# mitschabaude/msm-zprize

Measured on AMD Instinct MI355X. Metric: Mpoint-adds/s (ms per MSM in ms_per_step), higher is better.
Workload: dtype u32 limbs (28-bit lazy Montgomery, i64 accumulate)

## Files before the change

msm_zprize_amd/csrc/batch_kernels.h:

```cpp
#pragma once

namespace msmz {

#ifndef MSMZ_BATCH_BMAX
#define MSMZ_BATCH_BMAX 16
#endif
#ifdef MSMZ_EXP_NOMUL
#define BM_MUL(r, a, b) fe_add(r, a, b)
#define BM_SQR(r, a) fe_add(r, a, a)
#else
#define BM_MUL(r, a, b) fe_mul(r, a, b)
#define BM_SQR(r, a) fe_sqr(r, a)
#endif
enum { PK_NONE = 0, PK_ADD = 1, PK_DBL = 2, PK_TAKE_A = 3, PK_TAKE_B = 4, PK_INF = 5 };

template <class F, int T, bool SAFE, int OCC, int BMAX>
__global__ void __launch_bounds__(T, OCC) k_batch_add(uint32_t* slots, const uint32_t* points, const uint2* dsc,
                                                      uint32_t out_base, uint32_t total, int B, MsmMeta* meta) {
  __shared__ int32_t tree[F::N * T];
  __shared__ int32_t s_prev[F::N * T];
  __shared__ uint8_t s_kind[SAFE ? BMAX * T : 1];
  constexpr int N = F::N;
  const uint32_t block_base = blockIdx.x * (uint32_t)(T * B);
#ifdef MSMZ_TRACE
  uint64_t* trace = reinterpret_cast<uint64_t*>(meta + 1);
#endif
  MSMZ_STAMP(trace, 0);
  MSMZ_STAMP_HW(trace);

  Fe<F> prefix;
  fe_set_const<F>(prefix, F::ONE);
  int ilast = -1;
  if (block_base + threadIdx.x < total) {
    const uint32_t room = (total - 1u - block_base - threadIdx.x) / (uint32_t)T;
    ilast = room < (uint32_t)(B - 1) ? (int)room : B - 1;
  }
  uint2 dnext = make_uint2(0, 0);
  if (block_base + threadIdx.x < total) dnext = dsc[block_base + threadIdx.x];
#pragma unroll 1
  for (int i = 0; i < B; i++) {
    const uint32_t t = block_base + (uint32_t)i * T + threadIdx.x;
    uint32_t kind = PK_NONE;
    uint2 dd = dnext;
    if (i + 1 < B && t + (uint32_t)T < total) dnext = dsc[t + (uint32_t)T];
    if (t < total) {
#if defined(MSMZ_EXP_LOCALMEM) || defined(MSMZ_EXP_LOCAL_FWD)
      dd.x = LOC_ORIG | (t & 4095u);
      dd.y = LOC_ORIG | ((t + 1u) & 4095u);
#endif
      Fe<F> d;
      kind = PK_ADD;
      if constexpr (SAFE && SlotFmt<F>::PACKED) {
        Fe<F> x1, x2;
        const uint32_t oa = load_operand_x_or<F>(x1, dd.x, slots, points);
        const uint32_t ob = load_operand_x_or<F>(x2, dd.y, slots, points);
        fe_sub(d, x2, x1);
        if (oa == 0 || ob == 0 || fe_is_zero(d)) {
          Affine<F> p1, p2;
          const bool infA = load_operand<F, true>(p1, dd.x, slots, points);
          const bool infB = load_operand<F, true>(p2, dd.y, slots, points);
          if (infA) {
            kind = infB ? PK_INF : PK_TAKE_B;
          } else if (infB) {
            kind = PK_TAKE_A;
          } else if (fe_is_zero(d)) {
            Fe<F> num;
            fe_sub(num, p2.y, p1.y);
            if (fe_is_zero(num) && !fe_is_zero(p1.y)) {
              kind = PK_DBL;
              fe_add(d, p2.y, p2.y);
            } else {
// ... 208 lines not shown
```

msm_zprize_amd/csrc/engine.h:

```cpp
#pragma once
#include <hip/hip_runtime.h>

#include <chrono>
#include <cstdio>
#include <cstdlib>
#include <cstring>
#include <map>
#include <type_traits>
#include <vector>

#include "../../include/msmz.h"
#include "kernels.h"
#include "gen_kernels.h"
#include "import_kernels.h"
#include "check_kernels.h"
#include "mul_kernels.h"
#include "host64.h"
#include "multi.h"
#include "plan.h"

namespace msmz {

#define MSMZ_HIP(x)                                                                        \
  do {                                                                                     \
// ... 6 lines not shown

struct DevBuf {
  void* p = nullptr;
  size_t bytes = 0;
  DevBuf() = default;
  DevBuf(DevBuf&& o) noexcept : p(o.p), bytes(o.bytes) { o.p = nullptr, o.bytes = 0; }
  DevBuf& operator=(DevBuf&& o) noexcept {
    if (this != &o) {
      release();
      p = o.p, bytes = o.bytes;
      o.p = nullptr, o.bytes = 0;
    }
    return *this;
  }
  DevBuf(const DevBuf&) = delete;
  DevBuf& operator=(const DevBuf&) = delete;
  ~DevBuf() { release(); }
  int ensure(size_t need) {
    if (need <= bytes) return MSMZ_OK;
    release();
    size_t sz = need + need / 8;
    if (hipMalloc(&p, sz) != hipSuccess) {
      if (hipMalloc(&p, need) != hipSuccess) return MSMZ_ERR_HIP;
      sz = need;
    }
    bytes = sz;
    return MSMZ_OK;
  }
  void release() {
    if (p) (void)hipFree(p);
    p = nullptr;
    bytes = 0;
  }
  template <class T>
  T* as() const {
    return reinterpret_cast<T*>(p);
  }
};

struct Handle {
  int kind;
  uint64_t n;
  bool has_endo;
  DevBuf mem;
  uint32_t factor = 0;
  int c = 0, glv = 0;
  uint64_t copy_stride = 0;
  int sbits = 0;
};

struct StageEvents {
  hipEvent_t sort0, hist_end, scan_end, coarse_end, sort_end;
  hipEvent_t plan0, plan_end;
  hipEvent_t round_end[32];
  hipEvent_t acc_end, red_end;
  std::vector<hipEvent_t*> all() {
    std::vector<hipEvent_t*> v{&sort0, &hist_end, &scan_end, &coarse_end, &sort_end, &plan0, &plan_end, &acc_end, &red_end};
    for (hipEvent_t& e : round_end) v.push_back(&e);
    return v;
  }
};

struct Run {
  bool timing = false;
  StageEvents ev{};
  uint32_t max_bucket = 0, n_entries = 0, rounds = 0;
  uint32_t round_pairs[32] = {}, round_base[32] = {};
  uint64_t n_pairs = 0;
};

enum class Redo { NONE, PROVEN_BITS, PER_PROBLEM };

template <class F, bool TE>
static int host_point_add(const uint8_t* a, int ai, const uint8_t* b, int bi, uint8_t* out, int* oi) {
  constexpr int NW = F::NW;
  if constexpr (TE) {
    auto load = [](TeExt<F>& p, const uint8_t* xy) {
      uint32_t w[2 * NW];
      memcpy(w, xy, sizeof(w));
      Fe<F> x, y;
      fe_unpack<F>(x, w);
      fe_unpack<F>(y, w + NW);
      fe_to_mont(p.X, x);
      fe_to_mont(p.Y, y);
      fe_set_const<F>(p.Z, F::ONE);
      fe_mul(p.T, p.X, p.Y);
    };
    if (!a || !b) return MSMZ_ERR_ARG;
    TeExt<F> p, q, r;
    load(p, a);
    load(q, b);
    te_add(r, p, q);
    uint32_t w[2 * NW];
    te_to_affine_canon<F>(w, r);
    memcpy(out, w, sizeof(w));
    *oi = 0;
  } else {
    auto load = [](Xyzz<F>& p, const uint8_t* xy, int inf) {
      if (inf) {
        xyzz_set_inf(p);
        return;
      }
      uint32_t w[2 * NW];
      memcpy(w, xy, sizeof(w));
      Affine<F> t, m;
      fe_unpack<F>(t.x, w);
      fe_unpack<F>(t.y, w + NW);
      fe_to_mont(m.x, t.x);
      fe_to_mont(m.y, t.y);
      xyzz_from_affine(p, m);
    };
    Xyzz<F> p, q, r;
    load(p, a, ai);
    load(q, b, bi);
    xyzz_add(r, p, q);
    uint32_t w[2 * NW];
    bool inf = xyzz_to_affine_canon<F>(w, r);
    memcpy(out, w, sizeof(w));
    *oi = inf ? 1 : 0;
  }
  return MSMZ_OK;
}

struct ReduceKnobs {
  uint32_t tail_n;
  uint32_t quad16_max;
  uint32_t pairsum_x4_max;
};

template <class Cfg>
class TestHooks;

template <class Cfg>
class Engine : public IEngine {
  friend class TestHooks<Cfg>;
  using F = typename Cfg::F;
  using Fr = typename Cfg::Fr;
  static constexpr int NW = F::NW;
  static constexpr int RW = 2 * NW;
  static constexpr int XW = 4 * NW;
  static constexpr int FE_BYTES = NW * 4;
  static constexpr bool TE = Cfg::TE;
  static constexpr int PW_WORDS = TE ? 4 * NW : PointFmt<F>::STRIDE;

 public:
  Engine(int curve_id, int device) : curve_id_(curve_id), device_(device) {}

  int init() {
    MSMZ_HIP(hipSetDevice(device_));
    MSMZ_HIP(hipStreamCreateWithFlags(&stream_, hipStreamNonBlocking));
    for (hipEvent_t* e : ev_.all()) MSMZ_HIP(hipEventCreate(e));
    MSMZ_HIP(hipEventCreateWithFlags(&import_ev_, hipEventDisableTiming));
    MSMZ_HIP(hipHostMalloc(&h_meta_, sizeof(MsmMeta)));
    int st;
    if ((st = ensure_host_results((size_t)2 * kMaxWindows * XW))) return st;
    if ((st = raise_lds_limit((const void*)k_fine, "k_fine", kFineLds))) return st;
    if ((st = raise_sort_limits<false, 0>()) || (st = raise_sort_limits<false, 16>()) || (st = raise_sort_limits<false, 17>())) return st;
    if constexpr (Fr::HAS_GLV) {
      if ((st = raise_sort_limits<true, 0>()) || (st = raise_sort_limits<true, 16>())) return st;
    }
    return meta_.ensure(sizeof(MsmMeta) + kTraceBytes * 65536);
  }
 private:
  template <bool GLV, int C>
  int raise_sort_limits() {
    int st;
    if ((st = raise_lds_limit((const void*)k_coarse<Fr, GLV, C>, GLV ? "k_coarse<glv>" : "k_coarse", kCoarseLdsMax))) return st;
    return raise_lds_limit((const void*)k_hist<Fr, GLV, C>, GLV ? "k_hist<glv>" : "k_hist", kHistLdsMax);
  }
  static constexpr size_t kFineLds = ((size_t)(1 << FINE_MAX_BITS) + FINE_STAGE) * 4;
  static constexpr size_t kCoarseLdsMax = (size_t)2 * SORT_MAX_BINS * 4;
  static constexpr size_t kHistLdsMax = (size_t)SORT_MAX_BINS * 4;
#ifdef MSMZ_TRACE
  static constexpr size_t kTraceBytes = 128;
#else
  static constexpr size_t kTraceBytes = 0;
#endif

#ifdef MSMZ_TRACE
  int trace_dump(const char* name, const void* d_stamps, uint32_t n_wgs, bool first) {
    const char* path = getenv("MSMZ_TRACE_OUT");
    if (!path) return MSMZ_OK;
    MSMZ_HIP(hipStreamSynchronize(stream_));
    std::vector<uint64_t> t((size_t)n_wgs * 16);
    MSMZ_HIP(hipMemcpy(t.data(), d_stamps, t.size() * 8, hipMemcpyDeviceToHost));
    if (FILE* f = fopen(path, first ? "wb" : "ab")) {
      char nm[32] = {};
      strncpy(nm, name, 31);
      const uint64_t n = n_wgs;
      fwrite(nm, 1, 32, f);
      fwrite(&n, 8, 1, f);
      fwrite(t.data(), 8, t.size(), f);
      fclose(f);
    }
    return MSMZ_OK;
  }
#endif

  int raise_lds_limit(const void* fn, const char* name, size_t dyn_max) {
    hipFuncAttributes fa;
    memset(&fa, 0, sizeof(fa));
    MSMZ_HIP(hipFuncGetAttributes(&fa, fn));
    hipDeviceProp_t prop;
    MSMZ_HIP(hipGetDeviceProperties(&prop, device_));
    size_t dev_max = prop.sharedMemPerBlock;
    if (prop.sharedMemPerBlockOptin > dev_max) dev_max = prop.sharedMemPerBlockOptin;
    if (prop.maxSharedMemoryPerMultiProcessor > dev_max) dev_max = prop.maxSharedMemoryPerMultiProcessor;
    if (fa.sharedSizeBytes + dyn_max > dev_max) {
      fprintf(stderr, "msmz: %s needs %zu B static + %zu B dynamic LDS, the device offers %zu B per workgroup\n", name,
              (size_t)fa.sharedSizeBytes, dyn_max, dev_max);
      return MSMZ_ERR_HIP;
    }
    MSMZ_HIP(hipFuncSetAttribute(fn, hipFuncAttributeMaxDynamicSharedMemorySize, (int)dyn_max));
    return MSMZ_OK;
  }

 public:
  ~Engine() override {
    (void)hipSetDevice(device_);
    if (h_meta_) (void)hipHostFree(h_meta_);
    if (h_res_) (void)hipHostFree(h_res_);
    if (h_check_) (void)hipHostFree(h_check_);
    for (hipEvent_t* e : ev_.all())
      if (*e) (void)hipEventDestroy(*e);
    if (import_ev_) (void)hipEventDestroy(import_ev_);
    if (stream_) (void)hipStreamDestroy(stream_);
  }

  int upload_points(const uint8_t* xy, const uint8_t* inf, uint64_t n, uint64_t* h, const GenMap* split = nullptr) override {
    if (!xy || !h || n == 0 || n >= (1ull << (Cfg::HAS_ENDO ? 29 : 30))) return MSMZ_ERR_ARG;
    MSMZ_HIP(hipSetDevice(device_));
    int st = stage_.ensure(n * RW * 4 + n);
    if (st) return st;
    if ((st = copy_h2d(stage_.p, xy, (size_t)RW * 4, n, split))) return st;
    uint8_t* d_inf = nullptr;
    if (inf) {
      d_inf = stage_.as<uint8_t>() + n * RW * 4;
      if ((st = copy_h2d(d_inf, inf, 1, n, split))) return st;
    }
    const bool endo = Cfg::HAS_ENDO;
    Handle hd{0, n, endo};
    if ((st = alloc_handle(hd, (size_t)n * PW_WORDS * 4 * (endo ? 2 : 1)))) return st;
    MsmMeta* d_meta = meta_.as<MsmMeta>();
    MSMZ_HIP(hipMemsetAsync(&d_meta->error, 0, 4, stream_));
    if constexpr (TE) {
      hipLaunchKernelGGL((k_te_points_to_niels<F>), dim3((n + 255) / 256), dim3(256), 0, stream_, hd.mem.as<uint32_t>(),
                         stage_.as<uint32_t>(), (uint32_t)n, &d_meta->error);
    } else {
      hipLaunchKernelGGL((k_points_to_mont<F>), dim3((n + 255) / 256), dim3(256), 0, stream_, hd.mem.as<uint32_t>(),
                         stage_.as<uint32_t>(), d_inf, (uint32_t)n, endo ? 1 : 0, &d_meta->error);
    }
    uint32_t err = 0;
    if ((st = fetch_error(&err))) return st;
    if (err) return MSMZ_ERR_RANGE;
    return add_handle(std::move(hd), h);
  }

  int upload_scalars(const uint8_t* s, uint64_t n, uint64_t* h, const GenMap* split = nullptr) override {
    if (!s || !h || n == 0) return MSMZ_ERR_ARG;
    MSMZ_HIP(hipSetDevice(device_));
    Handle hd{1, n, false};
    int st;
    if ((st = alloc_handle(hd, n * 32)) || (st = copy_h2d(hd.mem.p, s, 32, n, split))) return st;
    MsmMeta* d_meta = meta_.as<MsmMeta>();
    MSMZ_HIP(hipMemsetAsync(&d_meta->error, 0, 4, stream_));
    hipLaunchKernelGGL((k_check_scalars<Fr>), dim3((n + 255) / 256), dim3(256), 0, stream_, &d_meta->error,
                       hd.mem.as<const uint32_t>(), (uint32_t)n);
    uint32_t err = 0;
    if ((st = fetch_error(&err))) return st;
    if (err) return MSMZ_ERR_RANGE;
    return add_handle(std::move(hd), h);
  }

  int import_scalars(const msmz_src& s, uint64_t n, uint64_t* h, const GenMap* split = nullptr) override {
    if (!h || n == 0 || n >> 32) return MSMZ_ERR_ARG;
    MSMZ_HIP(hipSetDevice(device_));
    Handle hd{1, n, false};
    ImportView v;
// ... 667 lines not shown
        hipLaunchKernelGGL(k_fine, dim3(fbins, P), dim3(FINE_T), lds, stream_, refs_.as<uint32_t>(), off_.as<uint32_t>(),
                           &d_meta->max_bucket, packed_.as<uint32_t>(), bins_.as<uint32_t>(), g.fb, g.fbt, sl.fine_top,
                           fbins, g.idx_bits, n_half, pl.endo_delta, g.F, g.mbits, copy_stride);
      }
#ifdef MSMZ_TRACE
      if ((st = trace_dump("k_coarse", tileoff_.as<uint32_t>() + (size_t)P * tiles * nbins, tiles, true))) return st;
      if ((st = trace_dump("k_fine", bins_.as<uint32_t>() + ((P * g.sbins + 2) & ~1u), fbins, false))) return st;
#endif
    } else {
      if (pl.fold_shift != 0) return MSMZ_ERR_ARG;
      if ((st = digits_.ensure((size_t)K * M * 4))) return st;
      if ((st = counts_.ensure(((size_t)nb + 1) * 4))) return st;
      if ((st = cursor_.ensure((size_t)nb * 4))) return st;
      if ((st = partials_.ensure((size_t)32 * nblocks * 4))) return st;
      MSMZ_HIP(hipMemsetAsync(counts_.p, 0, ((size_t)nb + 1) * 4, stream_));
      MSMZ_HIP(hipMemsetAsync(cursor_.p, 0, (size_t)nb * 4, stream_));
      const uint32_t dgrid = (n + 256 * DIGITS_ITEMS - 1) / (256 * DIGITS_ITEMS);
      mark(run, run.ev.sort0);
      if (pl.glv) {
        if constexpr (Fr::HAS_GLV)
          hipLaunchKernelGGL((k_digits<Fr, true>), dim3(dgrid), dim3(256), 0, stream_, digits_.as<uint32_t>(),
                             counts_.as<uint32_t>(), d_meta, d_scalars, n, c, K, pl.spread, pl.sbits ? pl.sbits : 256);
      } else {
        hipLaunchKernelGGL((k_digits<Fr, false>), dim3(dgrid), dim3(256), 0, stream_, digits_.as<uint32_t>(),
                           counts_.as<uint32_t>(), d_meta, d_scalars, n, c, K, pl.spread, pl.sbits ? pl.sbits : 256);
      }
      mark(run, run.ev.hist_end);
      MSMZ_HIP(hipGetLastError());
      hipLaunchKernelGGL(k_scan_partials, dim3(nblocks, 1), dim3(SCAN_T), 0, stream_, partials_.as<uint32_t>(),
                         counts_.as<uint32_t>(), nb, 0, nblocks);
      hipLaunchKernelGGL(k_scan_top, dim3(1), dim3(SCAN_T), 0, stream_, partials_.as<uint32_t>(), nblocks,
                         &d_meta->n_entries);
      hipLaunchKernelGGL(k_scan_apply, dim3(nblocks, 1), dim3(SCAN_T), 0, stream_, off_.as<uint32_t>(),
                         partials_.as<uint32_t>(), counts_.as<uint32_t>(), nb, 0, nblocks, (size_t)0,
                         &d_meta->max_bucket);
      mark(run, run.ev.scan_end);
      MSMZ_HIP(hipGetLastError());
      {
        dim3 grid((M + 256 * 4 - 1) / (256 * 4), K);
        hipLaunchKernelGGL(k_scatter, grid, dim3(256), 0, stream_, refs_.as<uint32_t>(), cursor_.as<uint32_t>(),
                           off_.as<uint32_t>(), digits_.as<uint32_t>(), M, c, pl.spread, n_half, pl.endo_delta);
      }
      mark(run, run.ev.coarse_end);
      MSMZ_HIP(hipGetLastError());
    }
    mark(run, run.ev.sort_end);
    MSMZ_HIP(hipGetLastError());
    return MSMZ_OK;
  }

  int fetch_meta(Run& run) {
    MSMZ_HIP(hipMemcpyAsync(h_meta_, meta_.p, sizeof(MsmMeta), hipMemcpyDeviceToHost, stream_));
    MSMZ_HIP(hipStreamSynchronize(stream_));
    run.max_bucket = h_meta_->max_bucket;
    run.n_entries = h_meta_->n_entries;
    run.rounds = h_meta_->rounds;
    memcpy(run.round_pairs, h_meta_->round_pairs, sizeof(run.round_pairs));
    memcpy(run.round_base, h_meta_->round_base, sizeof(run.round_base));
    return MSMZ_OK;
  }

  template <class P>
  int reduce_levels(const ReduceKnobs& rk, int& cur, uint32_t n_in, uint32_t nprob) {
    constexpr int AW = P::ACC_WORDS;
    int st;
    while (n_in > rk.tail_n) {
      const uint32_t S = 4;
      uint32_t g2 = (n_in + S - 1) / S;
      int nxt = cur ^ 1;
      if ((st = red_[nxt * 2].ensure((size_t)nprob * g2 * AW * 4))) return st;
      if ((st = red_[nxt * 2 + 1].ensure((size_t)nprob * g2 * AW * 4))) return st;
      uint32_t total = nprob * g2;
      if (total <= rk.quad16_max) {
        hipLaunchKernelGGL((k_reduce_quad16<P>), dim3((total * 16 + 63) / 64), dim3(64), 0, stream_,
                           red_[nxt * 2].as<uint32_t>(), red_[nxt * 2 + 1].as<uint32_t>(),
                           red_[cur * 2].as<uint32_t>(), red_[cur * 2 + 1].as<uint32_t>(), n_in, g2, total);
      } else {
        hipLaunchKernelGGL((k_reduce_quad<P>), dim3((total * 4 + 63) / 64), dim3(64), 0, stream_,
                           red_[nxt * 2].as<uint32_t>(), red_[nxt * 2 + 1].as<uint32_t>(),
                           red_[cur * 2].as<uint32_t>(), red_[cur * 2 + 1].as<uint32_t>(), n_in, g2, total);
      }
      n_in = g2;
      cur = nxt;
    }
    {
      const int nxt = cur ^ 1;
      if ((st = red_[nxt * 2].ensure((size_t)nprob * n_in * AW * 4))) return st;
      if ((st = red_[nxt * 2 + 1].ensure((size_t)nprob * n_in * AW * 4))) return st;
      if ((st = final_.ensure((size_t)nprob * AW * 4))) return st;
      hipLaunchKernelGGL((k_reduce_tail<P>), dim3(nprob), dim3(REDUCE_TAIL_T), 0, stream_, red_[cur * 2].as<uint32_t>(),
                         red_[cur * 2 + 1].as<uint32_t>(), red_[nxt * 2].as<uint32_t>(), red_[nxt * 2 + 1].as<uint32_t>(),
                         final_.as<uint32_t>(), n_in, n_in);
    }
    return MSMZ_OK;
  }

  int fetch_window_sums(const Plan& pl, size_t per_problem) {
    const size_t words = pl.nprob * per_problem * XW;
    if (int st = ensure_host_results(words)) return st;
    MSMZ_HIP(hipGetLastError());
    MSMZ_HIP(hipMemcpyAsync(h_res_, final_.p, words * 4, hipMemcpyDeviceToHost, stream_));
    MSMZ_HIP(hipMemcpyAsync(h_meta_, meta_.p, sizeof(MsmMeta), hipMemcpyDeviceToHost, stream_));
    MSMZ_HIP(hipStreamSynchronize(stream_));
    return MSMZ_OK;
  }

  struct HostTe {
    using Pt = TeExt<F>;
    void set_inf(Pt& p) const { te_set_zero(p); }
    void dbl(Pt& r, const Pt& p) const { te_add(r, p, p); }
    void add_pt(Pt& r, const Pt& a, const Pt& b) const { te_add(r, a, b); }
// ... 64 lines not shown
    } else if (basic) {
      hipLaunchKernelGGL((k_reduce2d_partial_acc<P>), dim3((total + 127) / 128), dim3(128), 0, stream_,
                         red_[0].as<uint32_t>(), slots_.as<uint32_t>(), rscan_.as<uint32_t>(), g, total);
    } else {
      if constexpr (!TE)
        hipLaunchKernelGGL((k_reduce2d_partial<F>), dim3((total + 127) / 128), dim3(128), 0, stream_,
                           red_[0].as<uint32_t>(), slots_.as<uint32_t>(), d_points, bfin_.as<uint4>(), g, total);
    }
    int src = 0;
    for (uint32_t n = total / 2; n >= lines && g.NC > 1; n /= 2) {
      const int dst = src ^ 2;
      if (n <= rk.pairsum_x4_max) {
        hipLaunchKernelGGL((k_pairsum_x4<P>), dim3((n * 4 + 63) / 64), dim3(64), 0, stream_, red_[dst].as<uint32_t>(),
                           red_[src].as<uint32_t>(), n);
      } else {
        hipLaunchKernelGGL((k_pairsum<P>), dim3((n + 127) / 128), dim3(128), 0, stream_, red_[dst].as<uint32_t>(),
                           red_[src].as<uint32_t>(), n);
      }
      src = dst;
      if (n == lines) break;
    }
    *rows = src;
    return MSMZ_OK;
  }
  template <class P>
  int weighted_sums_2d(const R2Geom& g, const ReduceKnobs& rk, int crow) {
    const uint32_t lines = g.nprob * g.H;
    const int ccol = crow + 1;
    int st;
    if ((st = red_[ccol].ensure((size_t)lines * XW * 4))) return st;
    hipLaunchKernelGGL((k_fill_neutral<P>), dim3((lines + 255) / 256), dim3(256), 0, stream_, red_[ccol].as<uint32_t>(), lines);
    int cur = crow >> 1;
    if ((st = reduce_levels<P>(rk, cur, g.H, g.nprob))) return st;
    MSMZ_HIP(hipGetLastError());
    return MSMZ_OK;
  }
  static void fill_log(msmz_log* log, const Plan& pl, const Run& run, float host_ms) {
    if (!log) return;
    log->c = pl.c;
    log->K = pl.K;
    log->rounds = (int)run.rounds;
    log->glv = pl.glv ? 1 : 0;
    log->n_entries = run.n_entries;
    log->n_pairs = run.n_pairs;
    log->max_bucket = run.max_bucket;
    log->stage_ms[MSMZ_ST_FINAL] = host_ms;
    if (!run.timing) return;
    const StageEvents& ev = run.ev;
    log->stage_ms[MSMZ_ST_DIGITS] = elapsed(ev.sort0, ev.hist_end);
    log->stage_ms[MSMZ_ST_SCAN] = elapsed(ev.hist_end, ev.scan_end);
    log->stage_ms[MSMZ_ST_SCATTER] = elapsed(ev.scan_end, ev.sort_end);
    log->scatter_kernel_ms = elapsed(ev.scan_end, ev.coarse_end);
    log->scatter_launches = 1;
    log->stage_ms[MSMZ_ST_PLAN] = elapsed(ev.plan0, ev.plan_end);
    log->stage_ms[MSMZ_ST_ACCUMULATE] = elapsed(ev.plan_end, ev.acc_end);
    log->stage_ms[MSMZ_ST_REDUCE] = elapsed(ev.acc_end, ev.red_end);
    hipEvent_t prev = ev.plan_end;
    for (uint32_t r = 0; r < run.rounds && r < 32; r++) {
      if (run.round_pairs[r] == 0) continue;
      log->batch_add_ms[r] = elapsed(prev, ev.round_end[r]);
      prev = ev.round_end[r];
    }
  }

  int plan_phase(const PlanChunks& pc, uint32_t nb, int tail_skip, size_t desc_records, Run& run) {
    int st;
    MsmMeta* d_meta = meta_.as<MsmMeta>();
    mark(run, run.ev.plan0);
    const uint32_t n_chunks = pc.n_main + (nb - pc.nb_main + pc.chunk_top - 1) / pc.chunk_top;
    const size_t pair_words = (size_t)n_chunks * (PLAN_RMAX - PLAN_RL) * PLAN_T;
    if ((st = rscan_.ensure(((size_t)PLAN_RMAX * n_chunks + pair_words) * 4 + kTraceBytes * n_chunks))) return st;
    if ((st = desc_.ensure(desc_records * 8))) return st;
    if ((st = bfin_.ensure((size_t)nb * 16))) return st;
    hipLaunchKernelGGL(k_plan_count, dim3(n_chunks), dim3(PLAN_T), 0, stream_, rscan_.as<uint32_t>(), off_.as<uint32_t>(),
                       nb, n_chunks, d_meta, tail_skip, pc);
    hipLaunchKernelGGL(k_plan_emit, dim3(n_chunks), dim3(PLAN_T), 0, stream_, desc_.as<uint2>(), bfin_.as<uint4>(),
                       d_meta, rscan_.as<uint32_t>(), off_.as<uint32_t>(), refs_.as<uint32_t>(), nb, n_chunks,
                       tail_skip, rscan_.as<uint32_t>() + (size_t)PLAN_RMAX * n_chunks, pc);
    MSMZ_HIP(hipGetLastError());
#ifdef MSMZ_TRACE
    if ((st = trace_dump("k_plan_emit", rscan_.as<uint32_t>() + (size_t)PLAN_RMAX * n_chunks + pair_words, n_chunks, false))) return st;
#endif
    return MSMZ_OK;
  }

  int msm_weierstrass_affine(const Handle& pts, const uint32_t* d_points, const uint32_t* d_scalars, uint64_t n64,
                             const msmz_opts& opt, uint8_t* out, int* out_inf, msmz_log* log, int extra_bits,
                             uint32_t nprob, Redo* redo) {
    const bool glv = opt.glv != 0;
    if (glv && (!Fr::HAS_GLV || !pts.has_endo)) return MSMZ_ERR_UNSUPPORTED;
    Plan pl;
    const bool want_2d = opt.reserved[0] != 1;
    const uint32_t fac = pts.factor > 1 ? pts.factor : 1;
    if (fac > 1 && (!want_2d || glv != (pts.glv != 0))) return MSMZ_ERR_UNSUPPORTED;
    int st = planner_.make_plan(pl, n64, glv, opt, (uint32_t)pts.n, true, extra_bits, want_2d, nprob, fac);
    if (st) return st;
    const SortLayout sl = planner_.sort_layout(pl);
    if (fac > 1 && !sl.two_level) return MSMZ_ERR_ARG;
    if (nprob > 1 && (!want_2d || !sl.two_level)) {
      *redo = Redo::PER_PROBLEM;
      return MSMZ_OK;
    }
    if ((uint64_t)nprob * pl.K * pl.M >= (1ull << 30)) return MSMZ_ERR_ARG;
    const size_t f2_records = opt.reserved[0] == 1 ? (size_t)13 * pl.Keff * ((pl.L + 1) / 2) + 256 : 0;
    if ((st = slots_.ensure(((size_t)nprob * pl.K * pl.M + 64 + f2_records) * SlotFmt<F>::WORDS * 4))) return st;
    Run run = new_run(opt);
    if ((st = sort_phase(pl, sl, d_scalars, run, (uint32_t)pts.copy_stride))) return st;
    const uint32_t nb = pl.nb * nprob;
    MsmMeta* d_meta = meta_.as<MsmMeta>();

    const int tail_skip = want_2d ? tail_skip_2d_ : 0;
    if ((st = plan_phase(planner_.plan_chunks(pl), nb, tail_skip, (size_t)nprob * pl.K * pl.M, run))) return st;
    if ((st = fetch_meta(run))) return st;
    if (h_meta_->error & 4u) return MSMZ_ERR_RANGE;
    if (h_meta_->error & 2u) {
      *redo = Redo::PROVEN_BITS;
      return MSMZ_OK;
    }
    if (run.max_bucket > (pl.F > 1 ? (1u << PLAN_RMAX) - 1u : (1u << 24))) return MSMZ_ERR_ARG;
    mark(run, run.ev.plan_end);
    const uint32_t R = run.rounds;
    for (uint32_t r = 0; r < R; r++) run.n_pairs += run.round_pairs[r];
    for (uint32_t r = 0; r < R; r++) {
      const uint32_t pairs = run.round_pairs[r];
      if (pairs == 0) continue;
      launch_batch_add(pairs, opt.safe != 0, d_points, desc_.as<uint2>() + run.round_base[r], run.round_base[r], d_meta);
#ifdef MSMZ_TRACE
      {
        char nm[32];
        snprintf(nm, sizeof nm, "k_batch_add round %d", r);
        const int B = batch_b(pairs);
        const uint32_t wgs = (pairs + MSMZ_BATCH_T * B - 1) / (MSMZ_BATCH_T * B);
        if ((st = trace_dump(nm, d_meta + 1, wgs < 65536 ? wgs : 65536, false))) return st;
      }
#endif
      mark(run, run.ev.round_end[r]);
    }
    mark(run, run.ev.acc_end);

    if (want_2d) {
      if ((st = reduce_2d<WeierPolicy<F>>(pl, planner_.split_2d(pl), reduce_knobs_, d_points))) return st;
    } else {
      uint32_t S1 = planner_.first_group_size(pl);
      if (S1 > 8) S1 = 8;
      while (S1 > 1 && S1 * 2 > pl.L) S1 >>= 1;
      const uint32_t groups = (pl.L + S1 - 1) / S1;
      if ((st = red_[0].ensure((size_t)pl.Keff * groups * XW * 4))) return st;
      if ((st = red_[1].ensure((size_t)pl.Keff * groups * XW * 4))) return st;
      if ((st = reduce_first_affine(pl, d_points, S1, groups, run.n_pairs, d_meta))) return st;
      int cur = 0;
      if ((st = reduce_levels<WeierPolicy<F>>(reduce_knobs_, cur, groups, (uint32_t)pl.Keff))) return st;
    }
    return finish_msm(pl, run, want_2d, out, out_inf, log);
  }

  int msm_basic(const Handle& pts, const uint32_t* d_points, const uint32_t* d_scalars, uint64_t n64, const msmz_opts& opt,
                uint8_t* out, int* out_inf, msmz_log* log) {
    using P = typename std::conditional<TE, TePolicy<F>, WeierPolicy<F>>::type;
    if (opt.glv) return MSMZ_ERR_UNSUPPORTED;
    Plan pl;
    int st = planner_.make_plan(pl, n64, false, opt, (uint32_t)pts.n, false);
    if (st) return st;
    Run run = new_run(opt);
    if ((st = sort_phase(pl, planner_.sort_layout(pl), d_scalars, run, 0)) || (st = fetch_meta(run))) return st;
    if (h_meta_->error & 4u) return MSMZ_ERR_RANGE;
    run.n_pairs = run.n_entries;
    if ((st = partials_.ensure((size_t)32 * pl.nblocks * 4))) return st;
    constexpr int AW = P::ACC_WORDS;
    const uint32_t nb = pl.nb, nblocks = pl.nblocks;
    MsmMeta* d_meta = meta_.as<MsmMeta>();
    mark(run, run.ev.plan0);
    int chunk_shift = chunk_shift_override_ > 0 ? chunk_shift_override_ : ACC_CHUNK_SHIFT;
    while ((1ull << (2 * chunk_shift)) < run.max_bucket) chunk_shift++;
    const int scan_mode = 2 | (chunk_shift << 4);
    if ((st = rscan_.ensure(((size_t)nb + 1) * 4))) return st;
    hipLaunchKernelGGL(k_scan_partials, dim3(nblocks, 1), dim3(SCAN_T), 0, stream_, partials_.as<uint32_t>(),
                       off_.as<uint32_t>(), nb, scan_mode, nblocks);
    hipLaunchKernelGGL(k_scan_top, dim3(1), dim3(SCAN_T), 0, stream_, partials_.as<uint32_t>(), nblocks,
                       d_meta->round_pairs);
    hipLaunchKernelGGL(k_scan_apply, dim3(nblocks, 1), dim3(SCAN_T), 0, stream_, rscan_.as<uint32_t>(),
                       partials_.as<uint32_t>(), off_.as<uint32_t>(), nb, scan_mode, nblocks, (size_t)0, (uint32_t*)nullptr);
    MSMZ_HIP(hipMemcpyAsync(h_meta_, d_meta, sizeof(MsmMeta), hipMemcpyDeviceToHost, stream_));
    MSMZ_HIP(hipStreamSynchronize(stream_));
    const uint32_t n_chunks = h_meta_->round_pairs[0];
    mark(run, run.ev.plan_end);
    if ((st = slots_.ensure((size_t)(n_chunks + 1) * AW * 4))) return st;
    if (n_chunks > 0) {
      hipLaunchKernelGGL((k_bucket_accumulate<P>), dim3((n_chunks + 127) / 128), dim3(128), 0, stream_,
                         slots_.as<uint32_t>(), d_points, refs_.as<uint32_t>(), off_.as<uint32_t>(),
// ... 25 lines not shown
    g.out0 = g.inf_slot + 64;
    uint32_t n_launch = 0, dsum = 0, osum = 0;
    for (uint32_t step = 1; step < S; step++) {
      g.ppg[n_launch] = 1;
      g.desc_off[n_launch] = dsum;
      g.out_off[n_launch] = osum;
      dsum += g.NG;
      osum += g.NG;
      n_launch++;
    }
    for (uint32_t n = S - 1; n > 1; n = n / 2 + (n & 1)) {
      g.ppg[n_launch] = n / 2;
      g.desc_off[n_launch] = dsum;
      g.out_off[n_launch] = osum;
      dsum += g.NG * (n / 2);
      osum += g.NG * (n / 2);
      n_launch++;
    }
    g.n_launches = n_launch;
    g.desc_off[n_launch] = dsum;
    dsum += g.NG;
    if ((uint64_t)g.out0 + osum + 64 >= (1ull << 30)) return MSMZ_ERR_ARG;
    int st;
    if ((st = f2desc_.ensure((size_t)dsum * 8))) return st;
    if (((size_t)g.out0 + osum + 64) * SlotFmt<F>::WORDS * 4 > slots_.bytes) return MSMZ_ERR_HIP;
    MSMZ_HIP(hipMemsetAsync(slots_.as<uint32_t>() + slot_words(g.inf_slot), 0, (size_t)64 * SlotFmt<F>::WORDS * 4, stream_));
    hipLaunchKernelGGL(k_reduce_affine_desc, dim3((g.NG + 255) / 256), dim3(256), 0, stream_, f2desc_.as<uint2>(),
                       bfin_.as<uint4>(), g);
    for (uint32_t i = 0; i < n_launch; i++)
      launch_batch_add(g.NG * g.ppg[i], true, d_points, f2desc_.as<uint2>() + g.desc_off[i], g.out0 + g.out_off[i], d_meta);
    hipLaunchKernelGGL((k_reduce_affine_finish<F>), dim3((g.NG + 127) / 128), dim3(128), 0, stream_, red_[0].as<uint32_t>(),
                       red_[1].as<uint32_t>(), slots_.as<uint32_t>(), d_points, f2desc_.as<uint2>() + g.desc_off[n_launch],
                       bfin_.as<uint4>(), g);
    MSMZ_HIP(hipGetLastError());
    return MSMZ_OK;
  }
  static size_t slot_words(uint32_t rec) {
    return (size_t)(rec >> 6) * (SlotFmt<F>::CH * 64) * 4;
  }

  int batch_b(uint32_t pairs) const {
    constexpr int T = MSMZ_BATCH_T, BMAX = MSMZ_BATCH_BMAX;
    int B = 1;
    while (B < BMAX && (uint64_t)pairs >= (uint64_t)T * (B * 2) * batch_min_wgs_) B *= 2;
    if (batch_b_override_ > 0) B = batch_b_override_ < BMAX ? batch_b_override_ : BMAX;
    return B;
  }

  void launch_batch_add(uint32_t pairs, bool safe, const uint32_t* d_points, const uint2* dsc, uint32_t out_base,
                        MsmMeta* d_meta) {
    launch_batch_add_b(batch_b(pairs), pairs, safe, d_points, dsc, out_base, d_meta);
  }
  void launch_batch_add_b(int B, uint32_t pairs, bool safe, const uint32_t* d_points, const uint2* dsc,
                          uint32_t out_base, MsmMeta* d_meta) {
    constexpr int T = MSMZ_BATCH_T, OCC = MSMZ_BATCH_OCC, BMAX = MSMZ_BATCH_BMAX;
    dim3 grid((pairs + T * B - 1) / (T * B)), block(T);
    if constexpr (!TE) {
      if (safe) {
        hipLaunchKernelGGL((k_batch_add<F, T, true, OCC, BMAX>), grid, block, 0, stream_, slots_.as<uint32_t>(),
                           d_points, dsc, out_base, pairs, B, d_meta);
      } else {
        hipLaunchKernelGGL((k_batch_add<F, T, false, OCC, BMAX>), grid, block, 0, stream_, slots_.as<uint32_t>(),
                           d_points, dsc, out_base, pairs, B, d_meta);
      }
    }
  }

  int ensure_gen_table() {
    if (gen_table_.p) return MSMZ_OK;
    int st = gen_table_.ensure((size_t)GEN_WINDOWS * GEN_TABLE * RW * 4);
    if (st) return st;
    uint32_t bases[GEN_WINDOWS * RW];
    Affine<F> ga;
    fe_set_const<F>(ga.x, F::GX);
    fe_set_const<F>(ga.y, F::GY);
    if constexpr (TE) {
      TeExt<F> g;
      g.X = ga.x;
      g.Y = ga.y;
      fe_set_const<F>(g.Z, F::ONE);
      fe_mul(g.T, ga.x, ga.y);
      for (int k = 0; k < GEN_WINDOWS; k++) {
        Fe<F> zi, x, y;
        fe_inverse(zi, g.Z);
        fe_mul(x, g.X, zi);
        fe_mul(y, g.Y, zi);
        fe_store<F>(bases + k * RW, x);
        fe_store<F>(bases + k * RW + NW, y);
        for (int j = 0; j < GEN_BITS; j++) {
          TeExt<F> t;
          te_add(t, g, g);
          g = t;
        }
      }
    } else {
      Xyzz<F> g;
      xyzz_from_affine(g, ga);
      for (int k = 0; k < GEN_WINDOWS; k++) {
        Affine<F> a;
        host_xyzz_to_affine_mont(a, g);
        fe_store<F>(bases + k * RW, a.x);
        fe_store<F>(bases + k * RW + NW, a.y);
        for (int j = 0; j < GEN_BITS; j++) {
          Xyzz<F> t;
          xyzz_dbl(t, g);
          g = t;
        }
      }
    }
    st = stage_.ensure(sizeof(bases));
    if (st) return st;
    MSMZ_HIP(hipMemcpyAsync(stage_.p, bases, sizeof(bases), hipMemcpyHostToDevice, stream_));
    if constexpr (TE) {
      hipLaunchKernelGGL((k_te_gen_table<F>), dim3((GEN_WINDOWS * GEN_TABLE + 127) / 128), dim3(128), 0, stream_,
                         gen_table_.as<uint32_t>(), stage_.as<uint32_t>());
    } else {
      hipLaunchKernelGGL((k_gen_table<F>), dim3((GEN_WINDOWS * GEN_TABLE + 127) / 128), dim3(128), 0, stream_,
                         gen_table_.as<uint32_t>(), stage_.as<uint32_t>());
    }
    MSMZ_HIP(hipGetLastError());
    MSMZ_HIP(hipStreamSynchronize(stream_));
    return MSMZ_OK;
  }

  static void host_xyzz_to_affine_mont(Affine<F>& a, const Xyzz<F>& p) {
    Fe<F> zi3, t, zi2;
    fe_inverse(zi3, p.ZZZ);
    fe_mul(t, zi3, p.ZZ);
    fe_sqr(zi2, t);
    fe_mul(a.x, p.X, zi2);
    fe_mul(a.y, p.Y, zi3);
  }

  int curve_id_, device_;
  hipStream_t stream_ = nullptr;
  StageEvents ev_{};
  hipEvent_t import_ev_ = nullptr;
  std::vector<uint8_t> import_pack_;
  std::map<uint64_t, Handle> handles_;
  uint64_t next_handle_ = 1;
#ifdef MSMZ_DEV
  static int env_int(const char* name, int dflt) { const char* v = getenv(name); return v ? atoi(v) : dflt; }
#else
  static int env_int(const char*, int dflt) { return dflt; }
#endif
  uint32_t batch_min_wgs_ = (uint32_t)env_int("MSMZ_BATCH_WGS", 512);
  int chunk_shift_override_ = env_int("MSMZ_CHUNK_SHIFT", 0);
  const ReduceKnobs reduce_knobs_{(uint32_t)env_int("MSMZ_TAIL_N", REDUCE_TAIL_N), (uint32_t)env_int("MSMZ_QUAD16", 8192),
                                  (uint32_t)env_int("MSMZ_PAIRSUM_X4", 16384)};
  Host64<F> host64_;
  bool no_bucket_sums_ = env_int("MSMZ_NO_BUCKET_SUMS", 0) != 0;
  int tail_skip_2d_ = env_int("MSMZ_TAIL_SKIP_2D", 1) > 2 ? 2 : env_int("MSMZ_TAIL_SKIP_2D", 1);
  int batch_b_override_ = env_int("MSMZ_BATCH_B", 0);
  int retries_ = 0;
  uint64_t pass_entries_ = kMaxEntriesPerPass;
  uint64_t range_passes_ = 0, sub_batches_ = 0;
  Planner<Fr> planner_{{env_int("MSMZ_NO_SPREAD", 0) != 0, env_int("MSMZ_NO_FOLD", 0) != 0,
                        env_int("MSMZ_NO_WINDOW_MODEL", 0) != 0, env_int("MSMZ_ATOMIC_SORT", 0) != 0,
                        env_int("MSMZ_NO_FBT", 0) != 0, env_int("MSMZ_NO_PLAN_TOP", 0) != 0,
                        env_int("MSMZ_NO_SORT_SPECIAL", 0) != 0, env_int("MSMZ_FB", 0), (uint32_t)env_int("MSMZ_S1", 0),
                        (uint32_t)env_int("MSMZ_R2_NC", 0)}};
  DevBuf bsum_, f2desc_, tilecnt_, tileoff_, final_, desc_, bfin_, packed_, bins_, digits_, counts_, off_, cursor_, refs_, rscan_, partials_, slots_, red_[4], meta_, stage_, gen_table_;
  MsmMeta* h_meta_ = nullptr;
  DevBuf check_;
  CheckResult* h_check_ = nullptr;
  size_t h_check_bytes_ = 0;
  int ensure_host_check(size_t verdict_bytes) {
    const size_t need = sizeof(CheckResult) + verdict_bytes;
    if (need <= h_check_bytes_) return MSMZ_OK;
    if (h_check_) (void)hipHostFree(h_check_);
    h_check_ = nullptr;
    h_check_bytes_ = 0;
    MSMZ_HIP(hipHostMalloc(&h_check_, need));
    h_check_bytes_ = need;
    return MSMZ_OK;
  }
  uint32_t* h_res_ = nullptr;
  size_t h_res_words_ = 0;
  int ensure_host_results(size_t words) {
    if (words <= h_res_words_) return MSMZ_OK;
    if (h_res_) (void)hipHostFree(h_res_);
    h_res_ = nullptr;
    h_res_words_ = 0;
    MSMZ_HIP(hipHostMalloc(&h_res_, words * 4));
    h_res_words_ = words;
    return MSMZ_OK;
  }
  TestHooks<Cfg> hooks_{*this};
};

// ... 2 lines not shown
```

msm_zprize_amd/csrc/instantiate.h:

```cpp
#pragma once
#include "check_kernels.h"
#include "gen_kernels.h"
#include "import_kernels.h"
#include "kernels.h"
#include "mul_kernels.h"
#include "test_kernels.h"

#if !defined(MSMZ_CURVE) || MSMZ_CURVE == 0
#define MSMZ_W0(X) X(Bls377Fp, Bls377Fr)
#else
#define MSMZ_W0(X)
#endif
#if !defined(MSMZ_CURVE) || MSMZ_CURVE == 1
#define MSMZ_W1(X) X(PallasFp, PallasFr)
#else
#define MSMZ_W1(X)
#endif
#if !defined(MSMZ_CURVE) || MSMZ_CURVE == 2
#define MSMZ_W2(X) X(Bls381Fp, Bls381Fr)
#else
#define MSMZ_W2(X)
#endif
#if !defined(MSMZ_CURVE) || MSMZ_CURVE == 3
#define MSMZ_T3(X) X(Ed377Fp, Ed377Fr)
#else
#define MSMZ_T3(X)
#endif
#define MSMZ_WEIERSTRASS_FIELDS(X) MSMZ_W0(X) MSMZ_W1(X) MSMZ_W2(X)
#define MSMZ_TE_FIELDS(X) MSMZ_T3(X)

#ifndef MSMZ_BATCH_T
#define MSMZ_BATCH_T 256
#endif
#ifndef MSMZ_BATCH_OCC
#define MSMZ_BATCH_OCC 4
#endif
#ifndef MSMZ_BATCH_BMAX
#define MSMZ_BATCH_BMAX 16
#endif

#define MSMZ_INST_BATCH(F, Fr, PFX)                                                                               \
  PFX template __global__ void k_batch_add<F, MSMZ_BATCH_T, true, MSMZ_BATCH_OCC, MSMZ_BATCH_BMAX>(              \
      uint32_t*, const uint32_t*, const uint2*, uint32_t, uint32_t, int, MsmMeta*);                              \
  PFX template __global__ void k_batch_add<F, MSMZ_BATCH_T, false, MSMZ_BATCH_OCC, MSMZ_BATCH_BMAX>(             \
      uint32_t*, const uint32_t*, const uint2*, uint32_t, uint32_t, int, MsmMeta*);

#define MSMZ_INST_POLICY(P, PFX)                                                                                 \
  PFX template __global__ void k_reduce_quad<P>(uint32_t*, uint32_t*, const uint32_t*, const uint32_t*, uint32_t, \
                                                uint32_t, uint32_t);                                             \
  PFX template __global__ void k_reduce_quad16<P>(uint32_t*, uint32_t*, const uint32_t*, const uint32_t*,        \
                                                  uint32_t, uint32_t, uint32_t);                                 \
  PFX template __global__ void k_reduce_tail<P>(uint32_t*, uint32_t*, uint32_t*, uint32_t*, uint32_t*, uint32_t, \
                                                uint32_t);                                                       \
  PFX template __global__ void k_pairsum<P>(uint32_t*, const uint32_t*, uint32_t);                               \
  PFX template __global__ void k_fill_neutral<P>(uint32_t*, uint32_t);                                           \
  PFX template __global__ void k_bucket_sums<P>(uint32_t*, const uint32_t*, const uint32_t*, uint32_t);          \
  PFX template __global__ void k_reduce2d_partial_acc<P>(uint32_t*, const uint32_t*, const uint32_t*, R2Geom, uint32_t); \
  PFX template __global__ void k_pairsum_x4<P>(uint32_t*, const uint32_t*, uint32_t);                            \
  PFX template __global__ void k_bucket_accumulate<P>(uint32_t*, const uint32_t*, const uint32_t*,               \
                                                      const uint32_t*, const uint32_t*, uint32_t, uint32_t, int);

#define MSMZ_INST_REDUCE(F, Fr, PFX)                                                                              \
  PFX template __global__ void k_reduce2d_partial<F>(uint32_t*, const uint32_t*, const uint32_t*, const uint4*,   \
                                                     R2Geom, uint32_t);                                          \
  PFX template __global__ void k_reduce_affine_finish<F>(uint32_t*, uint32_t*, const uint32_t*, const uint32_t*,  \
                                                         const uint2*, const uint4*, F2Geom);                     \
  MSMZ_INST_POLICY(WeierPolicy<F>, PFX)

#define MSMZ_INST_REDUCE_TE(F, Fr, PFX) MSMZ_INST_POLICY(TePolicy<F>, PFX)

#define MSMZ_INST_TEST(F, Fr, P, TE, PFX)                                                                         \
  PFX template __global__ void k_test_field<F>(uint32_t*, const uint32_t*, const uint32_t*, uint32_t, int, uint32_t*); \
  PFX template __global__ void k_test_field_limbs<F>(int32_t*, uint32_t*, const int32_t*, const int32_t*, uint32_t,  \
                                                      int, uint32_t*);                                            \
  PFX template __global__ void k_test_glv<Fr>(uint32_t*, uint32_t*, uint8_t*, const uint32_t*, uint32_t);         \
  PFX template __global__ void k_test_digits<Fr, false>(uint32_t*, const uint32_t*, uint32_t, int, int);          \
  PFX template __global__ void k_test_point<P, TE>(uint32_t*, const uint32_t*, const uint32_t*, const uint8_t*,   \
                                                   const uint8_t*, uint32_t, int);                                \
  PFX template __global__ void k_test_point_raw<P, TE>(uint32_t*, const uint32_t*, const uint32_t*, const uint8_t*, \
                                                       uint32_t, int, int);                                       \
  PFX template __global__ void k_test_accs_in<P, TE>(uint32_t*, const uint32_t*, const uint8_t*, const uint32_t*, \
                                                     uint32_t, uint32_t*);                                        \
  PFX template __global__ void k_test_accs_out<P, TE>(uint32_t*, const uint32_t*, uint32_t);

#define MSMZ_INST_SORT(Fr, GLV, C, PFX)                                                                           \
  PFX template __global__ void k_hist<Fr, GLV, C>(uint32_t*, uint16_t*, uint32_t*, MsmMeta*, const uint32_t*, SortGeom, uint32_t); \
  PFX template __global__ void k_coarse<Fr, GLV, C>(uint32_t*, const uint32_t*, const uint32_t*, const uint16_t*, const uint32_t*, SortGeom, uint32_t);

#define MSMZ_INST_SCALAR(Fr, PFX)                                                                                 \
  PFX template __global__ void k_digits<Fr, false>(uint32_t*, uint32_t*, MsmMeta*, const uint32_t*, uint32_t, int, int, int, int); \
  MSMZ_INST_SORT(Fr, false, 0, PFX)                                                                               \
  MSMZ_INST_SORT(Fr, false, 16, PFX)                                                                              \
  MSMZ_INST_SORT(Fr, false, 17, PFX)                                                                              \
  PFX template __global__ void k_check_scalars<Fr>(uint32_t*, const uint32_t*, uint32_t);                         \
  PFX template __global__ void k_gen_scalars<Fr>(uint32_t*, uint32_t, uint64_t, GenMap);                          \
  PFX template __global__ void k_import_scalars<Fr>(uint32_t*, const uint8_t*, uint64_t, int, uint32_t, int, uint32_t*);

#define MSMZ_INST_MISC(F, Fr, PFX)                                                                                \
// ... 37 lines not shown
```

Measured before the change: 4577.

## Launch round-0 batch add before host metadata readback, using device-side pair count

Result: no change. 4633 (median of 4 runs) (+1.2%).

```diff
diff --git a/msm_zprize_amd/csrc/batch_kernels.h b/msm_zprize_amd/csrc/batch_kernels.h
--- a/msm_zprize_amd/csrc/batch_kernels.h
+++ b/msm_zprize_amd/csrc/batch_kernels.h
@@ -16,7 +16,12 @@
 
 template <class F, int T, bool SAFE, int OCC, int BMAX>
 __global__ void __launch_bounds__(T, OCC) k_batch_add(uint32_t* slots, const uint32_t* points, const uint2* dsc,
-                                                      uint32_t out_base, uint32_t total, int B, MsmMeta* meta) {
+                                                      uint32_t out_base, uint32_t total, int B, MsmMeta* meta,
+                                                      const uint32_t* dev_total) {
+  if (dev_total) {
+    total = *dev_total;
+    if (blockIdx.x * (uint32_t)(T * B) >= total) return;
+  }
   __shared__ int32_t tree[F::N * T];
   __shared__ int32_t s_prev[F::N * T];
   __shared__ uint8_t s_kind[SAFE ? BMAX * T : 1];
diff --git a/msm_zprize_amd/csrc/engine.h b/msm_zprize_amd/csrc/engine.h
--- a/msm_zprize_amd/csrc/engine.h
+++ b/msm_zprize_amd/csrc/engine.h
@@ -82,10 +82,11 @@
 struct StageEvents {
   hipEvent_t sort0, hist_end, scan_end, coarse_end, sort_end;
   hipEvent_t plan0, plan_end;
+  hipEvent_t round0;
   hipEvent_t round_end[32];
   hipEvent_t acc_end, red_end;
   std::vector<hipEvent_t*> all() {
-    std::vector<hipEvent_t*> v{&sort0, &hist_end, &scan_end, &coarse_end, &sort_end, &plan0, &plan_end, &acc_end, &red_end};
+    std::vector<hipEvent_t*> v{&sort0, &hist_end, &scan_end, &coarse_end, &sort_end, &plan0, &plan_end, &round0, &acc_end, &red_end};
     for (hipEvent_t& e : round_end) v.push_back(&e);
     return v;
   }
@@ -93,6 +94,7 @@
 
 struct Run {
   bool timing = false;
+  bool round0_early = false;
   StageEvents ev{};
   uint32_t max_bucket = 0, n_entries = 0, rounds = 0;
   uint32_t round_pairs[32] = {}, round_base[32] = {};
@@ -181,6 +183,8 @@
     MSMZ_HIP(hipStreamCreateWithFlags(&stream_, hipStreamNonBlocking));
     for (hipEvent_t* e : ev_.all()) MSMZ_HIP(hipEventCreate(e));
     MSMZ_HIP(hipEventCreateWithFlags(&import_ev_, hipEventDisableTiming));
+    MSMZ_HIP(hipStreamCreateWithFlags(&copy_stream_, hipStreamNonBlocking));
+    MSMZ_HIP(hipEventCreateWithFlags(&meta_ev_, hipEventDisableTiming));
     MSMZ_HIP(hipHostMalloc(&h_meta_, sizeof(MsmMeta)));
     int st;
     if ((st = ensure_host_results((size_t)2 * kMaxWindows * XW))) return st;
@@ -254,6 +258,8 @@
     for (hipEvent_t* e : ev_.all())
       if (*e) (void)hipEventDestroy(*e);
     if (import_ev_) (void)hipEventDestroy(import_ev_);
+    if (meta_ev_) (void)hipEventDestroy(meta_ev_);
+    if (copy_stream_) (void)hipStreamDestroy(copy_stream_);
     if (stream_) (void)hipStreamDestroy(stream_);
   }
 
@@ -1027,11 +1033,22 @@
   int fetch_meta(Run& run) {
     MSMZ_HIP(hipMemcpyAsync(h_meta_, meta_.p, sizeof(MsmMeta), hipMemcpyDeviceToHost, stream_));
     MSMZ_HIP(hipStreamSynchronize(stream_));
+    read_meta(run);
+    return MSMZ_OK;
+  }
+  void read_meta(Run& run) {
     run.max_bucket = h_meta_->max_bucket;
     run.n_entries = h_meta_->n_entries;
     run.rounds = h_meta_->rounds;
     memcpy(run.round_pairs, h_meta_->round_pairs, sizeof(run.round_pairs));
     memcpy(run.round_base, h_meta_->round_base, sizeof(run.round_base));
+  }
+
+  int fetch_meta_aside(Run& run) {
+    MSMZ_HIP(hipStreamWaitEvent(copy_stream_, meta_ev_, 0));
+    MSMZ_HIP(hipMemcpyAsync(h_meta_, meta_.p, sizeof(MsmMeta), hipMemcpyDeviceToHost, copy_stream_));
+    MSMZ_HIP(hipStreamSynchronize(copy_stream_));
+    read_meta(run);
     return MSMZ_OK;
   }
 
@@ -1202,14 +1219,15 @@
     log->stage_ms[MSMZ_ST_SCATTER] = elapsed(ev.scan_end, ev.sort_end);
     log->scatter_kernel_ms = elapsed(ev.scan_end, ev.coarse_end);
     log->scatter_launches = 1;
-    log->stage_ms[MSMZ_ST_PLAN] = elapsed(ev.plan0, ev.plan_end);
-    log->stage_ms[MSMZ_ST_ACCUMULATE] = elapsed(ev.plan_end, ev.acc_end);
+    const hipEvent_t acc0 = run.round0_early ? ev.round0 : ev.plan_end;
+    log->stage_ms[MSMZ_ST_PLAN] = elapsed(ev.plan0, acc0);
+    log->stage_ms[MSMZ_ST_ACCUMULATE] = elapsed(acc0, ev.acc_end);
     log->stage_ms[MSMZ_ST_REDUCE] = elapsed(ev.acc_end, ev.red_end);
-    hipEvent_t prev = ev.plan_end;
+    hipEvent_t prev = acc0;
     for (uint32_t r = 0; r < run.rounds && r < 32; r++) {
       if (run.round_pairs[r] == 0) continue;
       log->batch_add_ms[r] = elapsed(prev, ev.round_end[r]);
-      prev = ev.round_end[r];
+      prev = r == 0 && run.round0_early ? ev.plan_end : ev.round_end[r];
     }
   }
 
@@ -1261,7 +1279,16 @@
 
     const int tail_skip = want_2d ? tail_skip_2d_ : 0;
     if ((st = plan_phase(planner_.plan_chunks(pl), nb, tail_skip, (size_t)nprob * pl.K * pl.M, run))) return st;
-    if ((st = fetch_meta(run))) return st;
+    MSMZ_HIP(hipEventRecord(meta_ev_, stream_));
+    const uint32_t r0_bound = (uint32_t)(((uint64_t)nprob * pl.K * pl.M) / 2);
+    const int r0_B = batch_b(r0_bound);
+    run.round0_early = true;
+    mark(run, run.ev.round0);
+    if (r0_bound > 0) {
+      launch_batch_add_b(r0_B, r0_bound, opt.safe != 0, d_points, desc_.as<uint2>(), 0, d_meta, d_meta->round_pairs);
+      mark(run, run.ev.round_end[0]);
+    }
+    if ((st = fetch_meta_aside(run))) return st;
     if (h_meta_->error & 4u) return MSMZ_ERR_RANGE;
     if (h_meta_->error & 2u) {
       *redo = Redo::PROVEN_BITS;
@@ -1274,17 +1301,17 @@
     for (uint32_t r = 0; r < R; r++) {
       const uint32_t pairs = run.round_pairs[r];
       if (pairs == 0) continue;
-      launch_batch_add(pairs, opt.safe != 0, d_points, desc_.as<uint2>() + run.round_base[r], run.round_base[r], d_meta);
+      if (r > 0) launch_batch_add(pairs, opt.safe != 0, d_points, desc_.as<uint2>() + run.round_base[r], run.round_base[r], d_meta);
 #ifdef MSMZ_TRACE
       {
         char nm[32];
         snprintf(nm, sizeof nm, "k_batch_add round %d", r);
-        const int B = batch_b(pairs);
+        const int B = r > 0 ? batch_b(pairs) : r0_B;
         const uint32_t wgs = (pairs + MSMZ_BATCH_T * B - 1) / (MSMZ_BATCH_T * B);
         if ((st = trace_dump(nm, d_meta + 1, wgs < 65536 ? wgs : 65536, false))) return st;
       }
 #endif
-      mark(run, run.ev.round_end[r]);
+      if (r > 0) mark(run, run.ev.round_end[r]);
     }
     mark(run, run.ev.acc_end);
 
@@ -1416,16 +1443,16 @@
     launch_batch_add_b(batch_b(pairs), pairs, safe, d_points, dsc, out_base, d_meta);
   }
   void launch_batch_add_b(int B, uint32_t pairs, bool safe, const uint32_t* d_points, const uint2* dsc,
-                          uint32_t out_base, MsmMeta* d_meta) {
+                          uint32_t out_base, MsmMeta* d_meta, const uint32_t* dev_pairs = nullptr) {
     constexpr int T = MSMZ_BATCH_T, OCC = MSMZ_BATCH_OCC, BMAX = MSMZ_BATCH_BMAX;
     dim3 grid((pairs + T * B - 1) / (T * B)), block(T);
     if constexpr (!TE) {
       if (safe) {
         hipLaunchKernelGGL((k_batch_add<F, T, true, OCC, BMAX>), grid, block, 0, stream_, slots_.as<uint32_t>(),
-                           d_points, dsc, out_base, pairs, B, d_meta);
+                           d_points, dsc, out_base, pairs, B, d_meta, dev_pairs);
       } else {
         hipLaunchKernelGGL((k_batch_add<F, T, false, OCC, BMAX>), grid, block, 0, stream_, slots_.as<uint32_t>(),
-                           d_points, dsc, out_base, pairs, B, d_meta);
+                           d_points, dsc, out_base, pairs, B, d_meta, dev_pairs);
       }
     }
   }
@@ -1500,6 +1527,8 @@
   hipStream_t stream_ = nullptr;
   StageEvents ev_{};
   hipEvent_t import_ev_ = nullptr;
+  hipStream_t copy_stream_ = nullptr;
+  hipEvent_t meta_ev_ = nullptr;
   std::vector<uint8_t> import_pack_;
   std::map<uint64_t, Handle> handles_;
   uint64_t next_handle_ = 1;
diff --git a/msm_zprize_amd/csrc/instantiate.h b/msm_zprize_amd/csrc/instantiate.h
--- a/msm_zprize_amd/csrc/instantiate.h
+++ b/msm_zprize_amd/csrc/instantiate.h
@@ -41,9 +41,9 @@
 
 #define MSMZ_INST_BATCH(F, Fr, PFX)                                                                               \
   PFX template __global__ void k_batch_add<F, MSMZ_BATCH_T, true, MSMZ_BATCH_OCC, MSMZ_BATCH_BMAX>(              \
-      uint32_t*, const uint32_t*, const uint2*, uint32_t, uint32_t, int, MsmMeta*);                              \
+      uint32_t*, const uint32_t*, const uint2*, uint32_t, uint32_t, int, MsmMeta*, const uint32_t*);               \
   PFX template __global__ void k_batch_add<F, MSMZ_BATCH_T, false, MSMZ_BATCH_OCC, MSMZ_BATCH_BMAX>(             \
-      uint32_t*, const uint32_t*, const uint2*, uint32_t, uint32_t, int, MsmMeta*);
+      uint32_t*, const uint32_t*, const uint2*, uint32_t, uint32_t, int, MsmMeta*, const uint32_t*);
 
 #define MSMZ_INST_POLICY(P, PFX)                                                                                 \
   PFX template __global__ void k_reduce_quad<P>(uint32_t*, uint32_t*, const uint32_t*, const uint32_t*, uint32_t, \
```
